# mpc001/auto_avsr

Hardware: AMD Instinct MI355X
Metric: video-frames/sec/node (25fps 88x88, max-frames=1600), E2E training step (fwd+bwd+clip+AdamW) (higher is better)
Workload: dtype f16 activations x f16x2 weights (atrunk3, atrunk4, decoder, encoder, trunk3, trunk4) + split-bf16 (everything else) forward / bf16 backward

## Files before the change

auto_avsr_amd/csrc/loss.hip:

```cpp
#include "prims.h"
#include "avsr_hip.h"
#include "ctc_common.h"

namespace {

AVSR_DEV float log_add(float a, float b) {
    const float m = fmaxf(a, b);
    if (m <= LOG_ZERO) return LOG_ZERO;
    return m + logf(avsr_exp(a - m) + avsr_exp(b - m));
}
AVSR_DEV float log_add3(float a, float b, float c) {
    const float m = fmaxf(a, fmaxf(b, c));
    if (m <= LOG_ZERO) return LOG_ZERO;
    const float sum = avsr_exp(a - m) + avsr_exp(b - m) + avsr_exp(c - m);
#ifdef AVSR_EMU
    return m + logf(sum);
#else
    return m + __logf(sum);
#endif
}

template <class T>
__global__ __launch_bounds__(256) void row_lse_kernel(const T* __restrict__ x, long ld, float* __restrict__ lse,
                                                      long rows, int V) {
// ... 310 lines not shown
    const uint64_t seed = seed0 + (seed_dev ? *seed_dev : 0ull);
    const float inv_keep = p > 0.f ? 1.f / (1.f - p) : 1.f;
    const int dv = D >> 3;
    for (long i = (long)blockIdx.x * 256 + threadIdx.x; i < rows * dv; i += (long)gridDim.x * 256) {
        const long r = i / dv;
        const int c = (int)(i % dv) * 8;
        float e[8], q[8], o[8];
        load8(table + ids[r] * D + c, e);
        load8(pe + (r % L) * D + c, q);
#pragma unroll
        for (int k = 0; k < 8; k++)
            o[k] = (e[k] * scale + q[k]) * dropout_scale(seed, (uint64_t)(r * D + c + k), p, inv_keep);
        store8(out + r * D + c, o);
    }
}
__global__ __launch_bounds__(256) void embed_bwd_kernel(const int64_t* __restrict__ ids, const float* __restrict__ dout,
                                                        float* __restrict__ dtable, long rows, int D, float scale,
                                                        float p, uint64_t seed0, const uint64_t* seed_dev) {
    const uint64_t seed = seed0 + (seed_dev ? *seed_dev : 0ull);
    const float inv_keep = p > 0.f ? 1.f / (1.f - p) : 1.f;
    for (long i = (long)blockIdx.x * 256 + threadIdx.x; i < rows * D; i += (long)gridDim.x * 256) {
        const long r = i / D;
        const int c = (int)(i % D);
        const int64_t id = ids[r];
        bool first = true;
        for (long q = 0; q < r; q++)
            if (ids[q] == id) {
                first = false;
                break;
            }
        if (!first) continue;
        float g = 0.f;
        for (long q = r; q < rows; q++)
// ... 95 lines not shown

extern "C" int avsr_embed_fwd(const int64_t* ids, const float* table, const float* pe, float* out, int64_t rows, int L,
                              int D, float scale, float drop_p, uint64_t seed, const uint64_t* seed_dev, hipStream_t stream) {
    AVSR_REQUIRE(D % 8 == 0, "embed: D must be a multiple of 8");
    if (rows <= 0) return 0;
    long nb = (rows * (D >> 3) + 255) / 256;
    AVSR_LAUNCH(embed_fwd_kernel, dim3((unsigned)(nb > 4096 ? 4096 : nb)), dim3(256), 0, stream, ids, table, pe, out, (long)rows, L, D, scale,
                drop_p, seed, seed_dev);
    AVSR_CHECK_LAUNCH("embed_fwd");
    return 0;
}

extern "C" int avsr_embed_bwd(const int64_t* ids, const float* dout, float* dtable, int64_t rows, int D, float scale,
                              float drop_p, uint64_t seed, const uint64_t* seed_dev, hipStream_t stream) {
    if (rows <= 0) return 0;
    long nb = (rows * D + 255) / 256;
    AVSR_LAUNCH(embed_bwd_kernel, dim3((unsigned)(nb > 4096 ? 4096 : nb)), dim3(256), 0, stream, ids, dout, dtable, (long)rows, D, scale, drop_p,
                seed, seed_dev);
    AVSR_CHECK_LAUNCH("embed_bwd");
    return 0;
}

extern "C" int avsr_log_softmax(const float* x, int64_t ld, float* lse_ws, float* out, int64_t rows, int V,
                                hipStream_t stream) {
    if (rows <= 0) return 0;
    int rc = avsr_row_lse(x, 0, ld, lse_ws, rows, V, stream);
    if (rc) return rc;
    AVSR_LAUNCH(sub_row_scalar_kernel, dim3((unsigned)rows), dim3(256), 0, stream, x, (long)ld, lse_ws, out, (long)rows, V);
    AVSR_CHECK_LAUNCH("log_softmax");
    return 0;
}
```

auto_avsr_amd/csrc/norm.hip:

```cpp
#include "prims.h"
#include "avsr_hip.h"

namespace {

constexpr int LN_THREADS = 256;
constexpr int LN_WAVES = LN_THREADS / 64;
constexpr int LN_MAXV = 4;

template <class TY>
__global__ __launch_bounds__(LN_THREADS) void layernorm_fwd_kernel(
    const float* __restrict__ x, const float* __restrict__ gamma, const float* __restrict__ beta,
    TY* __restrict__ y, float* __restrict__ mean_out, float* __restrict__ rstd_out, int rows,
    int cols, float eps, bf16_t* __restrict__ y2 = nullptr) {
    const int lane = threadIdx.x & 63;
    const int wave = threadIdx.x >> 6;
    const int row = blockIdx.x * LN_WAVES + wave;
    if (row >= rows) return;
    const float* xr = x + (size_t)row * cols;
    const int nvec = cols >> 3;
    float v[LN_MAXV][8];
    float s = 0.f;
#pragma unroll
    for (int i = 0; i < LN_MAXV; i++) {
        const int c = lane + 64 * i;
        if (c < nvec) {
            load8(xr + c * 8, v[i]);
#pragma unroll
            for (int e = 0; e < 8; e++) s += v[i][e];
        }
    }
    const float mean = wave_sum(s) / (float)cols;
    float q = 0.f;
#pragma unroll
    for (int i = 0; i < LN_MAXV; i++) {
        const int c = lane + 64 * i;
        if (c < nvec) {
#pragma unroll
            for (int e = 0; e < 8; e++) {
                const float d = v[i][e] - mean;
                q += d * d;
            }
        }
    }
    const float var = wave_sum(q) / (float)cols;
    const float rstd = 1.0f / sqrtf(var + eps);
    if (lane == 0) {
        mean_out[row] = mean;
        rstd_out[row] = rstd;
    }
    TY* yr = y + (size_t)row * cols;
#pragma unroll
    for (int i = 0; i < LN_MAXV; i++) {
        const int c = lane + 64 * i;
        if (c < nvec) {
            float g[8], b[8], o[8];
            load8(gamma + c * 8, g);
            load8(beta + c * 8, b);
#pragma unroll
            for (int e = 0; e < 8; e++) o[e] = (v[i][e] - mean) * rstd * g[e] + b[e];
            store8(yr + c * 8, o);
            if (y2) store8(y2 + (size_t)row * cols + c * 8, o);
        }
    }
}

template <class TDY>
AVSR_DEV void layernorm_bwd_dx_block(
    const TDY* __restrict__ dy, const float* __restrict__ x, const float* __restrict__ gamma,
    const float* __restrict__ mean_in, const float* __restrict__ rstd_in, const float* __restrict__ dres,
    float* __restrict__ dx, bf16_t* __restrict__ gout, float* __restrict__ gsum, float alpha0, float drop_p, uint64_t seed,
    int rows, int cols, int blk, int rpw, float* red) {
    const int lane = threadIdx.x & 63, wave = threadIdx.x >> 6;
    const int nvec = cols >> 3;
    const float inv_keep = drop_p > 0.f ? 1.f / (1.f - drop_p) : 1.f;
    float pc[LN_MAXV][8];
#pragma unroll
    for (int i = 0; i < LN_MAXV; i++)
#pragma unroll
// ... 171 lines not shown
    if (rows == 0) return 0;
    dim3 grid((rows + LN_WAVES - 1) / LN_WAVES), block(LN_THREADS);
    AVSR_LAUNCH((layernorm_fwd_kernel<float>), grid, block, 0, stream, x, gamma, beta, y, mean, rstd, rows, cols, eps, (bf16_t*)y2);
    AVSR_CHECK_LAUNCH("layernorm_fwd2");
    return 0;
}

extern "C" int avsr_layernorm_fwd_h16(const float* x, const float* gamma, const float* beta, void* y, void* y2, float* mean,
                                      float* rstd, int rows, int cols, float eps, hipStream_t stream) {
    AVSR_REQUIRE(cols % 8 == 0 && cols <= 64 * 8 * LN_MAXV, "layernorm: cols must be %8 and <= 2048");
    if (rows == 0) return 0;
    dim3 grid((rows + LN_WAVES - 1) / LN_WAVES), block(LN_THREADS);
    AVSR_LAUNCH((layernorm_fwd_kernel<f16_t>), grid, block, 0, stream, x, gamma, beta, (f16_t*)y, mean, rstd, rows, cols, eps,
                (bf16_t*)y2);
    AVSR_CHECK_LAUNCH("layernorm_fwd_h16");
    return 0;
}

extern "C" int avsr_layernorm_bwd(const void* dy, int dy_dtype, const float* x, const float* gamma,
                                  const float* mean, const float* rstd, const float* dres, float* dx,
                                  float* dgamma, float* dbeta, void* gout, float* gsum, float alpha, float drop_p,
                                  uint64_t seed, const uint64_t* seed_dev, int rows, int cols, hipStream_t stream) {
    AVSR_REQUIRE(cols % 8 == 0 && cols <= 64 * 8 * LN_MAXV, "layernorm: cols must be %8 and <= 2048");
    AVSR_REQUIRE(gsum == nullptr || gout != nullptr, "layernorm_bwd: gsum needs gout");
    if (rows == 0) return 0;
    float* gsum_det = nullptr;
    if (avsr_det() && gsum) {
        gsum_det = gsum;
        gsum = nullptr;
    }
// ... 20 lines not shown
```

auto_avsr_amd/csrc/optim.hip:

```cpp
#include <math.h>
#include "prims.h"
#include "avsr_hip.h"

namespace {

constexpr int OPT_CHUNK = 4096;

struct OptEntry {
    float* p;
    const float* g;
    float* m;
    float* v;
    long numel;
    int blk0, pad;
};

AVSR_DEV const OptEntry& find_entry(const OptEntry* table, int n, int blk) {
    int lo = 0, hi = n - 1;
    while (lo < hi) {
        const int mid = (lo + hi + 1) >> 1;
        if (table[mid].blk0 <= blk) lo = mid; else hi = mid - 1;
    }
    return table[lo];
}

struct AdamScalars {
    float coef, decay, step_size, inv_sqrt_bc2;
};
AVSR_DEV AdamScalars adam_scalars(const float* state, float beta1, float beta2, float weight_decay) {
    const float step = state[0], lr = state[1];
    const float bc1 = 1.f - powf(beta1, step), bc2 = 1.f - powf(beta2, step);
    return AdamScalars{state[3], 1.f - lr * weight_decay, lr / bc1, 1.f / sqrtf(bc2)};
}
AVSR_DEV void adam_update(float& p, float g, float& m, float& v, const AdamScalars& s, float beta1, float beta2, float eps) {
    const float gk = g * s.coef;
    p *= s.decay;
    m = beta1 * m + (1.f - beta1) * gk;
    v = beta2 * v + (1.f - beta2) * gk * gk;
    const float denom = sqrtf(v) * s.inv_sqrt_bc2 + eps;
// ... 64 lines not shown
        }
    }
}

__global__ __launch_bounds__(64) void grad_window_advance_kernel(float* __restrict__ window, float batch, int close) {
    if (blockIdx.x != 0 || threadIdx.x != 0) return;
    if (close) {
        window[0] = 0.f;
        window[1] = 0.f;
    } else {
        window[0] += 1.f;
        window[1] += batch;
    }
}

__global__ __launch_bounds__(256) void multi_sumsq_kernel(const OptEntry* __restrict__ table, int n, float* __restrict__ partial) {
    __shared__ float red[4];
    const OptEntry e = find_entry(table, n, blockIdx.x);
    const long base = (long)(blockIdx.x - e.blk0) * OPT_CHUNK;
    float s = 0.f;
#pragma unroll
    for (int j = 0; j < 4; j++) {
        const long i = base + (threadIdx.x + 256 * j) * 4;
        if (i + 3 < e.numel && (((uintptr_t)(e.g + i)) & 15) == 0) {
            const f32x4 g = *reinterpret_cast<const f32x4*>(e.g + i);
            s += g[0] * g[0] + g[1] * g[1] + g[2] * g[2] + g[3] * g[3];
        } else {
            for (int k = 0; k < 4; k++)
                if (i + k < e.numel) s += e.g[i + k] * e.g[i + k];
        }
    }
    s = wave_sum(s);
    if ((threadIdx.x & 63) == 0) red[threadIdx.x >> 6] = s;
    __syncthreads();
    if (threadIdx.x == 0) partial[blockIdx.x] = (red[0] + red[1]) + (red[2] + red[3]);
}

__global__ __launch_bounds__(1024) void clip_coef_kernel(const float* __restrict__ partial, int nparts, float max_norm,
                                                        float base_lr, float warmup_steps, float total_steps,
                                                        float* __restrict__ state) {
    __shared__ double red[16];
    double acc[8];
#pragma unroll
    for (int u = 0; u < 8; u++) acc[u] = 0.0;
    for (int i0 = threadIdx.x; i0 < nparts; i0 += 1024 * 8) {
        float v[8];
#pragma unroll
        for (int u = 0; u < 8; u++) v[u] = (i0 + 1024 * u < nparts) ? partial[i0 + 1024 * u] : 0.f;
#pragma unroll
        for (int u = 0; u < 8; u++) acc[u] += (double)v[u];
    }
    double s = ((acc[0] + acc[1]) + (acc[2] + acc[3])) + ((acc[4] + acc[5]) + (acc[6] + acc[7]));
    for (int m = 32; m >= 1; m >>= 1) s += __shfl_xor(s, m);
    if ((threadIdx.x & 63) == 0) red[threadIdx.x >> 6] = s;
    __syncthreads();
    if (threadIdx.x == 0) {
        double tot = 0.0;
        for (int w = 0; w < 16; w++) tot += red[w];
        const float norm = (float)sqrt(tot);
        const float step = state[0] + 1.f;
        float f;
        if (total_steps <= 0.f) f = 1.f;
        else if (step < warmup_steps) f = step / warmup_steps;
// ... 127 lines not shown
        }
#pragma unroll
        for (int k = 0; k < 8; k++) tile[(cc + k) * 72 + r] = f2bf(p[k]);
    }
    __syncthreads();
    if (e.dstT) {
        for (int id = threadIdx.x; id < 64 * 8; id += 256) {
            const int c = id >> 3, rr = (id & 7) * 8;
            const int gc = c0 + c, gr = r0 + rr;
            if (gc < e.C && gr < (e.limT ? e.limT : e.ldT))
                *reinterpret_cast<bf16x8*>(e.dstT + (long)gc * e.ldT + gr) = *reinterpret_cast<const bf16x8*>(tile + c * 72 + rr);
        }
    }
}

}

extern "C" int avsr_adamw_step(const void* table, int n, int total_blocks, float* partial, float* state, float base_lr,
                               float beta1, float beta2, float eps, float weight_decay, float max_grad_norm,
                               int64_t warmup_steps, int64_t total_steps, hipStream_t stream) {
    if (n <= 0 || total_blocks <= 0) return 0;
    AVSR_REQUIRE(table && partial && state, "adamw_step: null argument");
    const OptEntry* t = reinterpret_cast<const OptEntry*>(table);
    AVSR_LAUNCH(multi_sumsq_kernel, dim3(total_blocks), dim3(256), 0, stream, t, n, partial);
    AVSR_LAUNCH(clip_coef_kernel, dim3(1), dim3(1024), 0, stream, (const float*)partial, total_blocks, max_grad_norm, base_lr,
                (float)warmup_steps, (float)total_steps, state);
    AVSR_LAUNCH(multi_adamw_kernel, dim3(total_blocks), dim3(256), 0, stream, t, n, (const float*)state, beta1, beta2, eps,
                weight_decay);
    AVSR_CHECK_LAUNCH("adamw_step");
    return 0;
}

__global__ __launch_bounds__(1024) void sum_partials_kernel(const float* __restrict__ partial, int nparts, float* __restrict__ out) {
    __shared__ double red[16];
    double s = 0.0;
    for (int i = threadIdx.x; i < nparts; i += 1024) s += (double)partial[i];
    for (int m = 32; m >= 1; m >>= 1) s += __shfl_xor(s, m);
    if ((threadIdx.x & 63) == 0) red[threadIdx.x >> 6] = s;
    __syncthreads();
    if (threadIdx.x == 0) {
        double tot = 0.0;
        for (int w = 0; w < 16; w++) tot += red[w];
        out[0] = (float)tot;
    }
}
extern "C" int avsr_multi_sumsq(const void* table, int n, int total_blocks, float* partial, float* sumsq, hipStream_t stream) {
    AVSR_REQUIRE(table && partial && sumsq && n > 0 && total_blocks > 0, "multi_sumsq: bad arguments");
    AVSR_LAUNCH(multi_sumsq_kernel, dim3(total_blocks), dim3(256), 0, stream, reinterpret_cast<const OptEntry*>(table), n, partial);
    AVSR_LAUNCH(sum_partials_kernel, dim3(1), dim3(1024), 0, stream, (const float*)partial, total_blocks, sumsq);
    AVSR_CHECK_LAUNCH("multi_sumsq");
    return 0;
}
extern "C" int avsr_adamw_apply(const void* table, int n, int total_blocks, const float* sumsq, float* state, float base_lr,
                                float beta1, float beta2, float eps, float weight_decay, float max_grad_norm, int64_t warmup_steps,
                                int64_t total_steps, hipStream_t stream) {
    AVSR_REQUIRE(table && sumsq && state && n > 0 && total_blocks > 0, "adamw_apply: bad arguments");
    AVSR_LAUNCH(clip_coef_kernel, dim3(1), dim3(1024), 0, stream, sumsq, 1, max_grad_norm, base_lr, (float)warmup_steps,
                (float)total_steps, state);
    AVSR_LAUNCH(multi_adamw_kernel, dim3(total_blocks), dim3(256), 0, stream, reinterpret_cast<const OptEntry*>(table), n,
                (const float*)state, beta1, beta2, eps, weight_decay);
    AVSR_CHECK_LAUNCH("adamw_apply");
    return 0;
}

extern "C" int avsr_adamw_cast_step(const void* table, int n, int total_blocks, const void* lin_table, int lin_n,
                                    int lin_blocks, const void* tile_table, int tile_n, int tile_blocks, float* partial,
                                    float* state, float base_lr, float beta1, float beta2, float eps, float weight_decay,
                                    float max_grad_norm, int64_t warmup_steps, int64_t total_steps, hipStream_t stream) {
    if (n <= 0 || total_blocks <= 0) return 0;
    AVSR_REQUIRE(table && partial && state, "adamw_cast_step: null argument");
    AVSR_REQUIRE((lin_n <= 0 || lin_table) && (tile_n <= 0 || tile_table), "adamw_cast_step: null table");
    const OptEntry* t = reinterpret_cast<const OptEntry*>(table);
    AVSR_LAUNCH(multi_sumsq_kernel, dim3(total_blocks), dim3(256), 0, stream, t, n, partial);
    AVSR_LAUNCH(clip_coef_kernel, dim3(1), dim3(1024), 0, stream, (const float*)partial, total_blocks, max_grad_norm, base_lr,
                (float)warmup_steps, (float)total_steps, state);
    if (tile_n > 0 && tile_blocks > 0)
        AVSR_LAUNCH(multi_adamw_cast_kernel, dim3(tile_blocks), dim3(256), 0, stream,
                    reinterpret_cast<const OptTileEntry*>(tile_table), tile_n, (const float*)state, beta1, beta2, eps,
                    weight_decay);
    if (lin_n > 0 && lin_blocks > 0)
        AVSR_LAUNCH(multi_adamw_kernel, dim3(lin_blocks), dim3(256), 0, stream, reinterpret_cast<const OptEntry*>(lin_table),
                    lin_n, (const float*)state, beta1, beta2, eps, weight_decay);
    AVSR_CHECK_LAUNCH("adamw_cast_step");
    return 0;
}

extern "C" int avsr_multi_copy_scale(const void* table, int n, int total_blocks, float scale, hipStream_t stream) {
    if (n <= 0 || total_blocks <= 0) return 0;
    AVSR_LAUNCH(multi_copy_scale_kernel, dim3(total_blocks), dim3(256), 0, stream, reinterpret_cast<const OptEntry*>(table), n, scale);
    AVSR_CHECK_LAUNCH("multi_copy_scale");
// ... 14 lines not shown
```

auto_avsr_amd/functional.py:

```python
import contextlib
import os
import math
import struct
import weakref

import torch

from . import ops
from .ops import NN, NT, TN

_state = {"precise": False, "hpf": False, "mixed": False, "f16": False, "wp2": False, "seed": 0x5EED, "counter": 0, "seed_dev": None,
          "bn_sync": None}

MIXED_POLICY = {"encoder": "f16x2", "decoder": "f16x2", "trunk3": "f16x2", "trunk4": "f16x2", "atrunk3": "f16x2", "atrunk4": "f16x2"}
if os.environ.get("AVSR_MIXED_POLICY"):
    MIXED_POLICY = dict(kv.split("=") for kv in os.environ["AVSR_MIXED_POLICY"].split(",") if kv)


def set_precise(flag: bool):
    _state["precise"] = bool(flag)
    _state["hpf"] = _state["mixed"] = _state["f16"] = False
    ops.TWIN = None


# ... 899 lines not shown
    if t2 is None:
        ld = t.stride(-2)
        lead = t.shape[:-1]
        exp = ld
        for size, stride in zip(reversed(lead), reversed(t.stride()[:-1])):
            if size != 1 and stride != exp:
                return None
            exp *= size
        t2 = t.as_strided((rows, n), (ld, 1))
    ld = t2.stride(0)
    if ld % 8 or t2.data_ptr() % 16:
        return None
    return t2, ld


class LayerNormFn(torch.autograd.Function):

    @staticmethod
    def forward(ctx, x, gamma, beta, eps, out_dtype):
        x = x.contiguous()
        ctx.chain = _chain_take(x)
        y, mean, rstd = ops.layernorm_fwd(x, gamma, beta, out_dtype, eps)
        ctx.save_for_backward(x, gamma, mean, rstd)
        return y

    @staticmethod
    @_bwd_mode
    def backward(ctx, dy):
        x, gamma, mean, rstd = ctx.saved_tensors
        D = x.shape[-1]
        dg = _zeros(D, x.device)
        db = _zeros(D, x.device)
        dx = _ln_bwd(dy.contiguous(), x, gamma, mean, rstd, dg, db, None, ctx.chain)
        return dx, dg, db, None, None


def layer_norm(x, gamma, beta, eps=1e-12, out_dtype=torch.float32):
    _state["tag_ok"] = torch.is_grad_enabled()
    return LayerNormFn.apply(_to_f32(x), gamma, beta, eps, out_dtype)


class LinearFn(torch.autograd.Function):

    @staticmethod
    def forward(ctx, x, w, b, out_dtype, pad_out):
        x2 = x.contiguous()
        rows, K = _rows(x2), x2.shape[-1]
        N = w.shape[0]
        ldc = padded_cols(N) if pad_out else N
        alloc = torch.zeros if ldc != N else torch.empty
        y = alloc(x.shape[:-1] + (ldc,), dtype=out_dtype, device=x.device)
        _gemm_nt(x2, w, rows, N, K, y, ldc=ldc, bias=b)
        ctx.save_for_backward(_A(x2), w)
        ctx.meta = (b is not None, x.shape)
# ... 35 lines not shown

def linear(x, w, b=None, out_dtype=None, pad_out=False):
    _state["tag_ok"] = torch.is_grad_enabled()
    return LinearFn.apply(x, w, b, out_dtype or act_dtype(), pad_out)


class FfnSublayerFn(torch.autograd.Function):

    @staticmethod
    def forward(ctx, x, ln_w, ln_b, w1, b1, w2, b2, scale, p, eps):
        x = x.contiguous()
        ctx.chain = _chain_take(x)
        rows, D = _rows(x), x.shape[-1]
        Fh = w1.shape[0]
        T = act_dtype()
        h, mean, rstd = ops.layernorm_fwd(x, ln_w, ln_b, T, eps, twin=True)
        p1, s1, sd1 = _drop_args(p, x)
        u = torch.empty(rows, Fh, dtype=T, device=x.device)
        _gemm_nt(h, w1, rows, Fh, D, u, bias=b1, act=1, drop_p=p1, seed=s1, seed_dev=sd1, twin=True)
        p2, s2, sd2 = _drop_args(p, x)
        y = torch.empty_like(x)
        _gemm_nt(u, w2, rows, D, Fh, y, bias=b2, drop_p=p2, seed=s2, seed_dev=sd2, alpha=scale, resid=x, ldr=D)
        ctx.save_for_backward(x, ln_w, mean, rstd, _A(h), _A(u), w1, w2)
        ctx.meta = (scale, p1, p2, s2, sd2)
        _chain_tag(y, rows, D, scale, (p2, s2, sd2))
        return y

    @staticmethod
    @_bwd_mode
    def backward(ctx, dy):
        x, ln_w, mean, rstd, h, u, w1, w2 = ctx.saved_tensors
# ... 98 lines not shown
        dx = torch.empty(x2.shape, dtype=torch.float32, device=g.device)
        with ops.paired():
            dw1 = _wgrad(du, x2, rows, Fh, Din)
            _gemm_nn(du, w1, rows, Din, Fh, dx)
        return dx, dw1, db1, dw2, db2


def mlp(x, w1, b1, w2, b2):
    _state["tag_ok"] = torch.is_grad_enabled()
    return MlpFn.apply(x, w1, b1, w2, b2)


from .functional_convmod import (
    _const_cache, _const1, _bn_train_stats, _bn_bwd_sums, ConvSublayerFn, conv_sublayer)
from .functional_attention import (
    prepare_pos_proj, _placeholders, _placeholder_grad, PosProjFn, _proj, AttentionCoreFn, attention_core,
    MhaSublayerFn, mha_sublayer, MemoryKVFn, memory_kv)
from .functional_heads import (
    ScaleDropoutFn, scale_dropout, EmbedFn, embed, CtcLossFn, ctc_loss, ctc_align, ctc_beam_search, ctc_score, CeSmoothFn,
    ce_smooth, AddRowsFn, add, log_softmax)
from .functional_frontend import (
    _bn_fwd_params, _bn_bwd, bn_tuple, BasicBlockFn, basic_block, StemFn, stem, AvgPoolFn, avg_pool, trunk_1d)
```

auto_avsr_amd/functional_attention.py:

```python
import math

import torch

from . import functional as AF
from . import ops
from .functional import (
    _A, _A_shared, _A_view, _bgrad, _bias3, _bwd_mode, _chain_tag, _chain_take, _drop_args, _gemm_nn, _gemm_nt,
    _ln_bwd, _mask_arg, _pos_proj, _prologue, _state, _to_act, _to_act_shared, _to_f32, _w_bf16_cat, _w_h16_cat, _h16_nt,
    _wgrad, _zeros, act_dtype)


def prepare_pos_proj(pos_emb, weights):
    _pos_proj.clear()
    if _state["precise"] or len(weights) < 2 or pos_emb is None:
        return
    D = pos_emb.shape[-1]
    if D % 64 or any(w.dtype != torch.float32 or not w.is_contiguous() or tuple(w.shape) != (D, D) for w in weights):
        return
    pe = _to_act_shared(pos_emb).reshape(-1, D)
    if pe.dtype not in (torch.bfloat16, torch.float16):
        return
    n, P = len(weights), pe.shape[0]
    if torch.is_grad_enabled() and all(w.requires_grad for w in weights):
        holder = {}
# ... 13 lines not shown
def _shared_pos_proj(pos_emb, wpos):
    ent = _pos_proj.get(pos_emb, wpos)
    return ent[1] if ent is not None else (None,) * 4


_placeholders = {}


def _placeholder_grad(shape, dtype, device):
    z = _placeholders.get((dtype, device))
    if z is None:
        z = _placeholders[(dtype, device)] = torch.zeros((), dtype=dtype, device=device)
    return z.expand(shape)


class PosProjFn(torch.autograd.Function):

    @staticmethod
    def forward(ctx, pos_emb, holder, *weights):
        D = pos_emb.shape[-1]
        pe = _to_act_shared(pos_emb).reshape(-1, D)
        n, P = len(weights), pe.shape[0]
        out = torch.empty(P, n * D, dtype=pe.dtype, device=pe.device)
        if pe.dtype == torch.float16:
            _h16_nt(pe, D, _w_h16_cat(tuple(weights)), P, n * D, D, out, n * D, planes=1, twin=True)
        else:
            ops.gemm_bf16_nt(pe, D, _w_bf16_cat(tuple(weights), False), D, P, n * D, D, out, n * D)
        ctx.save_for_backward(_A_shared(pe))
        ctx.holder, ctx.meta = holder, (P, D, n)
        return out

    @staticmethod
    @_bwd_mode
    def backward(ctx, dout):
        (pe,) = ctx.saved_tensors
        P, D, n = ctx.meta
        holder = ctx.holder
        assert holder.get("filled", 0) == n and holder.get("dpos") is not None, \
            "PosProjFn: every encoder layer must have accumulated its position gradient"
        dW = _wgrad(holder["dpos"], pe, P, n * D, D)
        holder["dpos"] = None
        holder["filled"] = 0
        return (None, None) + tuple(dW[i * D:(i + 1) * D] for i in range(n))



def _proj(h, w, b, rows, D, twin=True):
    out = torch.empty(rows, w.shape[0], dtype=act_dtype(), device=h.device)
    _gemm_nt(h, w, rows, w.shape[0], D, out, bias=b, twin=twin)
    return out


class AttentionCoreFn(torch.autograd.Function):

    @staticmethod
# ... 376 lines not shown
```

auto_avsr_amd/nets.py:

```python
import math

import torch
from torch import nn

from . import functional as AF
from .scorer_interface import BatchScorerInterface


class LayerNorm(nn.LayerNorm):

    def __init__(self, nout, dim=-1):
        super().__init__(nout, eps=1e-12)
        self.dim = dim

    def forward(self, x):
        if self.dim == -1:
            return AF.layer_norm(x, self.weight, self.bias, self.eps)
        return AF.layer_norm(x.transpose(1, -1), self.weight, self.bias, self.eps).transpose(1, -1)


class PositionwiseFeedForward(nn.Module):

    def __init__(self, idim, hidden_units, dropout_rate):
        super().__init__()
        self.w_1 = nn.Linear(idim, hidden_units)
        self.w_2 = nn.Linear(hidden_units, idim)
        self.dropout = nn.Dropout(dropout_rate)

    def forward(self, x):
        p = self.dropout.p if self.training else 0.0
        return AF.ffn(x, self.w_1.weight, self.w_1.bias, self.w_2.weight, self.w_2.bias, p)

# ... 204 lines not shown
        self.conv_module = conv_module
        self.macaron_style = macaron_style
        self.norm_ff = LayerNorm(size)
        self.norm_mha = LayerNorm(size)
        if macaron_style:
            self.feed_forward_macaron = copy.deepcopy(feed_forward)
            self.ff_scale = 0.5
            self.norm_ff_macaron = LayerNorm(size)
        if conv_module is not None:
            self.norm_conv = LayerNorm(size)
            self.norm_final = LayerNorm(size)
        self.dropout = nn.Dropout(dropout_rate)
        self.size = size
        self.normalize_before = normalize_before
        self.concat_after = concat_after

    def _ffn(self, x, norm, ff):
        p = self.dropout.p if self.training else 0.0
        return AF.ffn_sublayer(x, norm.weight, norm.bias, ff.w_1.weight, ff.w_1.bias, ff.w_2.weight, ff.w_2.bias,
                               self.ff_scale, p, norm.eps)

    def forward(self, x_input, mask, cache=None):
        if cache is not None:
            raise NotImplementedError("incremental encoder cache (dead code in the reference, SURVEY F10)")
        x, pos_emb = x_input if isinstance(x_input, tuple) else (x_input, None)
        p = self.dropout.p if self.training else 0.0
        if self.macaron_style:
            x = self._ffn(x, self.norm_ff_macaron, self.feed_forward_macaron)
        a = self.self_attn
        relpos = pos_emb is not None
        x = AF.mha_sublayer(x, None, pos_emb, mask, self.norm_mha.weight, self.norm_mha.bias, *a._params(),
                            a.linear_pos.weight if relpos else None, a.pos_bias_u if relpos else None,
                            a.pos_bias_v if relpos else None, a.h, a._p_attn(), p, self.norm_mha.eps)
        if self.conv_module is not None:
            x = AF.conv_sublayer(x, self.norm_conv.weight, self.norm_conv.bias, *self.conv_module._params(), p,
                                 self.norm_conv.eps)
        x = self._ffn(x, self.norm_ff, self.feed_forward)
        if self.conv_module is not None:
            x = self.norm_final(x)
        return ((x, pos_emb), mask) if relpos else (x, mask)


def _rename(state_dict, old, new):
    for k in [k for k in state_dict if k.startswith(old)]:
        state_dict[new + k[len(old):]] = state_dict.pop(k)


def _encoder_legacy_keys(state_dict, prefix, *_):
    _rename(state_dict, prefix + "input_layer.", prefix + "embed.")
    _rename(state_dict, prefix + "norm.", prefix + "after_norm.")


class ConformerEncoder(nn.Module):

# ... 5 lines not shown
        self._register_load_state_dict_pre_hook(_encoder_legacy_keys)
        self.embed = nn.Sequential(RelPositionalEncoding(attention_dim, positional_dropout_rate))
        self.normalize_before = normalize_before
        self.encoders = repeat(
            num_blocks,
            lambda n: EncoderLayer(
                attention_dim,
                RelPositionMultiHeadedAttention(attention_heads, attention_dim, attention_dropout_rate, zero_triu),
                PositionwiseFeedForward(attention_dim, linear_units, dropout_rate),
                ConvolutionModule(attention_dim, cnn_module_kernel) if use_cnn_module else None,
                dropout_rate, normalize_before, concat_after, macaron_style),
            layer_drop_rate=0.0,
        )
        if normalize_before:
            self.after_norm = LayerNorm(attention_dim)

    def forward(self, xs, masks):
        with AF.component("encoder"):
            xs = self.embed(xs)
            if isinstance(xs, tuple):
                AF.prepare_pos_proj(xs[1], [layer.self_attn.linear_pos.weight for layer in self.encoders
                                            if hasattr(layer.self_attn, "linear_pos")])
            xs, masks = self.encoders(xs, masks)
            if isinstance(xs, tuple):
                xs = xs[0]
            if self.normalize_before:
                xs = self.after_norm(xs)
        return xs, masks

    def forward_one_step(self, xs, masks, cache=None):
# ... 296 lines not shown
```

auto_avsr_amd/ops.py:

```python
import contextlib
import math
import os

import torch

from . import _lib

F32, BF16, F16 = 0, 1, 2
_DT = {torch.float32: F32, torch.bfloat16: BF16, torch.float16: F16}
NT, NN, TN = 0, 1, 2


def dt(t, split8_ok=False):
    if isinstance(t, Split8):
        if not split8_ok:
            raise TypeError("a split8-layout activation reached an entry point that cannot read it")
        return 3
    return _DT[t.dtype]


def _ptr(t):
    return None if t is None else t.data_ptr()


# ... 91 lines not shown
    y = torch.empty(x.shape, dtype=out_dtype, device=x.device)
    mean = torch.empty(rows, dtype=torch.float32, device=x.device)
    rstd = torch.empty(rows, dtype=torch.float32, device=x.device)
    y2 = _twin(y) if twin else None
    if out_dtype == torch.float16:
        call("avsr_layernorm_fwd_h16", _ptr(x), _ptr(gamma), _ptr(beta), _ptr(y), _ptr(y2), _ptr(mean), _ptr(rstd), rows, cols, eps,
             _stream(x), nbytes=_nb(x, y, y2))
        return y, mean, rstd
    if y2 is not None:
        call("avsr_layernorm_fwd2", _ptr(x), _ptr(gamma), _ptr(beta), _ptr(y), _ptr(y2), _ptr(mean), _ptr(rstd), rows, cols, eps,
             _stream(x), nbytes=_nb(x, y, y2))
        return y, mean, rstd
    call("avsr_layernorm_fwd", _ptr(x), _ptr(gamma), _ptr(beta), _ptr(y), dt(y), _ptr(mean), _ptr(rstd),
         rows, cols, eps, _stream(x), nbytes=_nb(x, y))
    return y, mean, rstd


def layernorm_bwd(dy, x, gamma, mean, rstd, dgamma, dbeta, dres=None, gout=None, gsum=None, alpha=1.0, drop_p=0.0,
                  seed=0, seed_dev=None):
    rows, cols = x.numel() // x.shape[-1], x.shape[-1]
    dx = torch.empty_like(x)
    call("avsr_layernorm_bwd", _ptr(dy), dt(dy), _ptr(x), _ptr(gamma), _ptr(mean), _ptr(rstd), _ptr(dres),
         _ptr(dx), _ptr(dgamma), _ptr(dbeta), _ptr(gout), _ptr(gsum), alpha, drop_p, seed, _ptr(seed_dev), rows, cols,
         _stream(x), nbytes=_nb(dy, x, dres, dx, gout))
    return dx


def gemm(layout, A, lda, B, ldb, M, N, K, C, ldc, *, precise=False, bias=None, act=0, gate=None, ldg=0,
         gate_scale=1.0, drop_p=0.0, seed=0, seed_dev=None, alpha=1.0, alpha_dev=None, resid=None, ldr=0,
         accumulate=False, split_k=1, force_tile=0):
# ... 873 lines not shown
```

include/avsr_hip.h:

```cpp
#ifndef AVSR_HIP_H
#define AVSR_HIP_H
#include <stdint.h>

#if defined(__HIP__) || defined(AVSR_EMU)
typedef hipStream_t avsr_stream_t;
#else
typedef void* avsr_stream_t;
#endif

#ifdef __cplusplus
extern "C" {
#endif

int avsr_abi_version(void);
int avsr_is_emulator(void);
const char* avsr_last_error(void);

int avsr_layernorm_fwd(const float* x, const float* gamma, const float* beta, void* y, int y_dtype,
                       float* mean, float* rstd, int rows, int cols, float eps,
                       avsr_stream_t stream);
int avsr_layernorm_fwd2(const float* x, const float* gamma, const float* beta, float* y, void* y2, float* mean, float* rstd,
                        int rows, int cols, float eps, avsr_stream_t stream);
int avsr_layernorm_bwd(const void* dy, int dy_dtype, const float* x, const float* gamma,
                       const float* mean, const float* rstd, const float* dres, float* dx,
                       float* dgamma, float* dbeta, void* gout, float* gsum, float alpha, float drop_p, uint64_t seed,
                       const uint64_t* seed_dev, int rows, int cols, avsr_stream_t stream);

int avsr_gemm(int layout, const void* A, int a_dtype, int lda, const void* B, int b_dtype, int ldb,
              int M, int N, int K, int precise, const float* bias, int act, const void* gate,
              int gate_dtype, int ldg, float gate_scale, float drop_p, uint64_t seed, const uint64_t* seed_dev,
              float alpha, const float* alpha_dev, const float* resid, int ldr, void* C, int c_dtype, int ldc,
              int accumulate, int split_k, int force_tile, avsr_stream_t stream);

int avsr_attention_fwd(const void* qu, const void* qv, const void* k, const void* v, const void* pos,
                       int dtype, int precise, const uint8_t* mask, int64_t mask_sb, int64_t mask_sq,
                       void* out, float* lse, int B, int H, int Tq, int Tk, int dk, int ldq, int ldk,
                       int ldv, int ldp, int ldo, int64_t sbq, int64_t sbk, int64_t sbv, int64_t sbo,
// ... 342 lines not shown
```

Before: 70520.

## Fuse back-to-back layernorms, rework embed backward and grad-norm reduction

Adds a paired layernorm kernel that computes the encoder layer's final norm and the next layer's macaron FFN norm (or the after_norm) from a single read of the row, handing the second result over through a cache. The embedding backward now has each block build a shared-memory bitmask of rows with matching ids instead of every thread rescanning all earlier ids. The gradient sum-of-squares uses fewer walker blocks that accumulate in double precision. The positional-projection weight gradient casts dpos to bf16 first. These cut launches and redundant memory traffic, at the cost of hand-off state in Python and extra code paths.

```diff
diff --git a/auto_avsr_amd/csrc/loss.hip b/auto_avsr_amd/csrc/loss.hip
--- a/auto_avsr_amd/csrc/loss.hip
+++ b/auto_avsr_amd/csrc/loss.hip
@@ -348,9 +348,61 @@
         store8(out + r * D + c, o);
     }
 }
+constexpr long EMBED_BWD_MAX_ROWS = 32768;
 __global__ __launch_bounds__(256) void embed_bwd_kernel(const int64_t* __restrict__ ids, const float* __restrict__ dout,
                                                         float* __restrict__ dtable, long rows, int D, float scale,
                                                         float p, uint64_t seed0, const uint64_t* seed_dev) {
+    AVSR_DYN_SMEM(smem);
+    const uint64_t seed = seed0 + (seed_dev ? *seed_dev : 0ull);
+    const float inv_keep = p > 0.f ? 1.f / (1.f - p) : 1.f;
+    const int nw = (int)((rows + 63) >> 6);
+    uint64_t* words = reinterpret_cast<uint64_t*>(smem);
+    uint8_t* flag = reinterpret_cast<uint8_t*>(words + nw);
+    for (long r = blockIdx.x; r < rows; r += gridDim.x) {
+        const int64_t id = ids[r];
+        for (int q = threadIdx.x; q < nw * 64; q += 256) flag[q] = (uint8_t)(q < rows && ids[q] == id);
+        __syncthreads();
+        for (int w = threadIdx.x; w < nw; w += 256) {
+            uint64_t m = 0;
+#pragma unroll 8
+            for (int k = 0; k < 64; k++) m |= (uint64_t)flag[w * 64 + k] << k;
+            words[w] = m;
+        }
+        __syncthreads();
+        const int wr = (int)(r >> 6);
+        const uint64_t below = (1ull << (r & 63)) - 1ull;
+        bool first = (words[wr] & below) == 0;
+        for (int w = 0; w < wr && first; w++) first = words[w] == 0;
+        if (first)
+            for (int c = threadIdx.x; c < D; c += 256) {
+                float g = 0.f;
+                for (int w = wr; w < nw; w++) {
+                    uint64_t m = w == wr ? words[w] & ~below : words[w];
+                    while (m) {
+                        long q[4];
+                        float d[4];
+                        int nq = 0;
+#pragma unroll
+                        for (int k = 0; k < 4; k++)
+                            if (m) {
+                                q[nq++] = (long)w * 64 + __builtin_ctzll(m);
+                                m &= m - 1;
+                            }
+#pragma unroll
+                        for (int k = 0; k < 4; k++) d[k] = k < nq ? dout[q[k] * D + c] : 0.f;
+#pragma unroll
+                        for (int k = 0; k < 4; k++)
+                            if (k < nq) g += d[k] * scale * dropout_scale(seed, (uint64_t)(q[k] * D + c), p, inv_keep);
+                    }
+                }
+                dtable[id * D + c] += g;
+            }
+        __syncthreads();
+    }
+}
+__global__ __launch_bounds__(256) void embed_bwd_scan_kernel(const int64_t* __restrict__ ids, const float* __restrict__ dout,
+                                                             float* __restrict__ dtable, long rows, int D, float scale,
+                                                             float p, uint64_t seed0, const uint64_t* seed_dev) {
     const uint64_t seed = seed0 + (seed_dev ? *seed_dev : 0ull);
     const float inv_keep = p > 0.f ? 1.f / (1.f - p) : 1.f;
     for (long i = (long)blockIdx.x * 256 + threadIdx.x; i < rows * D; i += (long)gridDim.x * 256) {
@@ -476,9 +528,15 @@
 extern "C" int avsr_embed_bwd(const int64_t* ids, const float* dout, float* dtable, int64_t rows, int D, float scale,
                               float drop_p, uint64_t seed, const uint64_t* seed_dev, hipStream_t stream) {
     if (rows <= 0) return 0;
-    long nb = (rows * D + 255) / 256;
-    AVSR_LAUNCH(embed_bwd_kernel, dim3((unsigned)(nb > 4096 ? 4096 : nb)), dim3(256), 0, stream, ids, dout, dtable, (long)rows, D, scale, drop_p,
-                seed, seed_dev);
+    if (rows <= EMBED_BWD_MAX_ROWS) {
+        const size_t lds = (size_t)((rows + 63) / 64) * 72;
+        AVSR_LAUNCH(embed_bwd_kernel, dim3((unsigned)(rows > 4096 ? 4096 : rows)), dim3(256), lds, stream, ids, dout, dtable, (long)rows, D,
+                    scale, drop_p, seed, seed_dev);
+    } else {
+        long nb = (rows * D + 255) / 256;
+        AVSR_LAUNCH(embed_bwd_scan_kernel, dim3((unsigned)(nb > 4096 ? 4096 : nb)), dim3(256), 0, stream, ids, dout, dtable, (long)rows, D,
+                    scale, drop_p, seed, seed_dev);
+    }
     AVSR_CHECK_LAUNCH("embed_bwd");
     return 0;
 }
diff --git a/auto_avsr_amd/csrc/norm.hip b/auto_avsr_amd/csrc/norm.hip
--- a/auto_avsr_amd/csrc/norm.hip
+++ b/auto_avsr_amd/csrc/norm.hip
@@ -6,6 +6,57 @@
 constexpr int LN_THREADS = 256;
 constexpr int LN_WAVES = LN_THREADS / 64;
 constexpr int LN_MAXV = 4;
+
+template <class TY, bool KEEP>
+AVSR_DEV void layernorm_row(float (&v)[LN_MAXV][8], int lane, int nvec, int cols, const float* __restrict__ gamma,
+                            const float* __restrict__ beta, float eps, TY* __restrict__ yr, bf16_t* __restrict__ y2r,
+                            float* __restrict__ mean_out, float* __restrict__ rstd_out) {
+    float s = 0.f;
+#pragma unroll
+    for (int i = 0; i < LN_MAXV; i++) {
+        const int c = lane + 64 * i;
+        if (c < nvec) {
+#pragma unroll
+            for (int e = 0; e < 8; e++) s += v[i][e];
+        }
+    }
+    const float mean = wave_sum(s) / (float)cols;
+    float q = 0.f;
+#pragma unroll
+    for (int i = 0; i < LN_MAXV; i++) {
+        const int c = lane + 64 * i;
+        if (c < nvec) {
+#pragma unroll
+            for (int e = 0; e < 8; e++) {
+                const float d = v[i][e] - mean;
+                q += d * d;
+            }
+        }
+    }
+    const float var = wave_sum(q) / (float)cols;
+    const float rstd = 1.0f / sqrtf(var + eps);
+    if (lane == 0) {
+        *mean_out = mean;
+        *rstd_out = rstd;
+    }
+#pragma unroll
+    for (int i = 0; i < LN_MAXV; i++) {
+        const int c = lane + 64 * i;
+        if (c < nvec) {
+            float g[8], b[8], o[8];
+            load8(gamma + c * 8, g);
+            load8(beta + c * 8, b);
+#pragma unroll
+            for (int e = 0; e < 8; e++) o[e] = (v[i][e] - mean) * rstd * g[e] + b[e];
+            store8(yr + c * 8, o);
+            if (y2r) store8(y2r + c * 8, o);
+            if (KEEP) {
+#pragma unroll
+                for (int e = 0; e < 8; e++) v[i][e] = o[e];
+            }
+        }
+    }
+}
 
 template <class TY>
 __global__ __launch_bounds__(LN_THREADS) void layernorm_fwd_kernel(
@@ -19,49 +70,36 @@
     const float* xr = x + (size_t)row * cols;
     const int nvec = cols >> 3;
     float v[LN_MAXV][8];
-    float s = 0.f;
-#pragma unroll
-    for (int i = 0; i < LN_MAXV; i++) {
-        const int c = lane + 64 * i;
-        if (c < nvec) {
-            load8(xr + c * 8, v[i]);
-#pragma unroll
-            for (int e = 0; e < 8; e++) s += v[i][e];
-        }
-    }
-    const float mean = wave_sum(s) / (float)cols;
-    float q = 0.f;
-#pragma unroll
-    for (int i = 0; i < LN_MAXV; i++) {
-        const int c = lane + 64 * i;
-        if (c < nvec) {
-#pragma unroll
-            for (int e = 0; e < 8; e++) {
-                const float d = v[i][e] - mean;
-                q += d * d;
-            }
-        }
-    }
-    const float var = wave_sum(q) / (float)cols;
-    const float rstd = 1.0f / sqrtf(var + eps);
-    if (lane == 0) {
-        mean_out[row] = mean;
-        rstd_out[row] = rstd;
-    }
-    TY* yr = y + (size_t)row * cols;
-#pragma unroll
-    for (int i = 0; i < LN_MAXV; i++) {
-        const int c = lane + 64 * i;
-        if (c < nvec) {
-            float g[8], b[8], o[8];
-            load8(gamma + c * 8, g);
-            load8(beta + c * 8, b);
-#pragma unroll
-            for (int e = 0; e < 8; e++) o[e] = (v[i][e] - mean) * rstd * g[e] + b[e];
-            store8(yr + c * 8, o);
-            if (y2) store8(y2 + (size_t)row * cols + c * 8, o);
-        }
-    }
+#pragma unroll
+    for (int i = 0; i < LN_MAXV; i++) {
+        const int c = lane + 64 * i;
+        if (c < nvec) load8(xr + c * 8, v[i]);
+    }
+    layernorm_row<TY, false>(v, lane, nvec, cols, gamma, beta, eps, y + (size_t)row * cols,
+                             y2 ? y2 + (size_t)row * cols : nullptr, mean_out + row, rstd_out + row);
+}
+
+template <class TH>
+__global__ __launch_bounds__(LN_THREADS) void layernorm_fwd_pair_kernel(
+    const float* __restrict__ x, const float* __restrict__ gamma1, const float* __restrict__ beta1, float* __restrict__ y,
+    float* __restrict__ mean1, float* __restrict__ rstd1, float eps1, const float* __restrict__ gamma2,
+    const float* __restrict__ beta2, TH* __restrict__ h, bf16_t* __restrict__ h2, float* __restrict__ mean2,
+    float* __restrict__ rstd2, float eps2, int rows, int cols) {
+    const int lane = threadIdx.x & 63;
+    const int wave = threadIdx.x >> 6;
+    const int row = blockIdx.x * LN_WAVES + wave;
+    if (row >= rows) return;
+    const float* xr = x + (size_t)row * cols;
+    const int nvec = cols >> 3;
+    float v[LN_MAXV][8];
+#pragma unroll
+    for (int i = 0; i < LN_MAXV; i++) {
+        const int c = lane + 64 * i;
+        if (c < nvec) load8(xr + c * 8, v[i]);
+    }
+    layernorm_row<float, true>(v, lane, nvec, cols, gamma1, beta1, eps1, y + (size_t)row * cols, nullptr, mean1 + row, rstd1 + row);
+    layernorm_row<TH, false>(v, lane, nvec, cols, gamma2, beta2, eps2, h + (size_t)row * cols,
+                             h2 ? h2 + (size_t)row * cols : nullptr, mean2 + row, rstd2 + row);
 }
 
 template <class TDY>
@@ -263,6 +301,26 @@
     AVSR_LAUNCH((layernorm_fwd_kernel<f16_t>), grid, block, 0, stream, x, gamma, beta, (f16_t*)y, mean, rstd, rows, cols, eps,
                 (bf16_t*)y2);
     AVSR_CHECK_LAUNCH("layernorm_fwd_h16");
+    return 0;
+}
+
+extern "C" int avsr_layernorm_fwd_pair(const float* x, const float* gamma1, const float* beta1, float* y, float* mean1, float* rstd1,
+                                       float eps1, const float* gamma2, const float* beta2, void* h, int h_dtype, void* h2,
+                                       float* mean2, float* rstd2, float eps2, int rows, int cols, hipStream_t stream) {
+    AVSR_REQUIRE(cols % 8 == 0 && cols <= 64 * 8 * LN_MAXV, "layernorm: cols must be %8 and <= 2048");
+    AVSR_REQUIRE(h_dtype >= 0 && h_dtype <= 2, "layernorm_fwd_pair: h_dtype is 0 (f32), 1 (bf16) or 2 (f16)");
+    if (rows == 0) return 0;
+    dim3 grid((rows + LN_WAVES - 1) / LN_WAVES), block(LN_THREADS);
+    if (h_dtype == 0)
+        AVSR_LAUNCH((layernorm_fwd_pair_kernel<float>), grid, block, 0, stream, x, gamma1, beta1, y, mean1, rstd1, eps1, gamma2, beta2,
+                    (float*)h, (bf16_t*)h2, mean2, rstd2, eps2, rows, cols);
+    else if (h_dtype == 1)
+        AVSR_LAUNCH((layernorm_fwd_pair_kernel<bf16_t>), grid, block, 0, stream, x, gamma1, beta1, y, mean1, rstd1, eps1, gamma2, beta2,
+                    (bf16_t*)h, (bf16_t*)h2, mean2, rstd2, eps2, rows, cols);
+    else
+        AVSR_LAUNCH((layernorm_fwd_pair_kernel<f16_t>), grid, block, 0, stream, x, gamma1, beta1, y, mean1, rstd1, eps1, gamma2, beta2,
+                    (f16_t*)h, (bf16_t*)h2, mean2, rstd2, eps2, rows, cols);
+    AVSR_CHECK_LAUNCH("layernorm_fwd_pair");
     return 0;
 }
 
diff --git a/auto_avsr_amd/csrc/optim.hip b/auto_avsr_amd/csrc/optim.hip
--- a/auto_avsr_amd/csrc/optim.hip
+++ b/auto_avsr_amd/csrc/optim.hip
@@ -15,14 +15,15 @@
     int blk0, pad;
 };
 
-AVSR_DEV const OptEntry& find_entry(const OptEntry* table, int n, int blk) {
+AVSR_DEV int find_index(const OptEntry* table, int n, int blk) {
     int lo = 0, hi = n - 1;
     while (lo < hi) {
         const int mid = (lo + hi + 1) >> 1;
         if (table[mid].blk0 <= blk) lo = mid; else hi = mid - 1;
     }
-    return table[lo];
-}
+    return lo;
+}
+AVSR_DEV const OptEntry& find_entry(const OptEntry* table, int n, int blk) { return table[find_index(table, n, blk)]; }
 
 struct AdamScalars {
     float coef, decay, step_size, inv_sqrt_bc2;
@@ -117,29 +118,55 @@
     }
 }
 
+AVSR_DEV float chunk_sumsq(const float* __restrict__ g, long numel, long base) {
+    float s = 0.f;
+#pragma unroll
+    for (int j = 0; j < 4; j++) {
+        const long i = base + (threadIdx.x + 256 * j) * 4;
+        if (i + 3 < numel && (((uintptr_t)(g + i)) & 15) == 0) {
+            const f32x4 v = *reinterpret_cast<const f32x4*>(g + i);
+            s += v[0] * v[0] + v[1] * v[1] + v[2] * v[2] + v[3] * v[3];
+        } else {
+            for (int k = 0; k < 4; k++)
+                if (i + k < numel) s += g[i + k] * g[i + k];
+        }
+    }
+    return s;
+}
+
 __global__ __launch_bounds__(256) void multi_sumsq_kernel(const OptEntry* __restrict__ table, int n, float* __restrict__ partial) {
     __shared__ float red[4];
     const OptEntry e = find_entry(table, n, blockIdx.x);
-    const long base = (long)(blockIdx.x - e.blk0) * OPT_CHUNK;
-    float s = 0.f;
-#pragma unroll
-    for (int j = 0; j < 4; j++) {
-        const long i = base + (threadIdx.x + 256 * j) * 4;
-        if (i + 3 < e.numel && (((uintptr_t)(e.g + i)) & 15) == 0) {
-            const f32x4 g = *reinterpret_cast<const f32x4*>(e.g + i);
-            s += g[0] * g[0] + g[1] * g[1] + g[2] * g[2] + g[3] * g[3];
-        } else {
-            for (int k = 0; k < 4; k++)
-                if (i + k < e.numel) s += e.g[i + k] * e.g[i + k];
-        }
-    }
+    float s = chunk_sumsq(e.g, e.numel, (long)(blockIdx.x - e.blk0) * OPT_CHUNK);
     s = wave_sum(s);
     if ((threadIdx.x & 63) == 0) red[threadIdx.x >> 6] = s;
     __syncthreads();
     if (threadIdx.x == 0) partial[blockIdx.x] = (red[0] + red[1]) + (red[2] + red[3]);
 }
 
-__global__ __launch_bounds__(1024) void clip_coef_kernel(const float* __restrict__ partial, int nparts, float max_norm,
+constexpr int SUMSQ_WALKERS = 2048;
+__global__ __launch_bounds__(256) void multi_sumsq_walk_kernel(const OptEntry* __restrict__ table, int n, int total_blocks,
+                                                               double* __restrict__ partial) {
+    __shared__ double red[4];
+    const int per = (total_blocks + (int)gridDim.x - 1) / (int)gridDim.x;
+    const int b0 = (int)blockIdx.x * per;
+    const int b1 = b0 + per < total_blocks ? b0 + per : total_blocks;
+    double s = 0.0;
+    if (b0 < b1) {
+        int idx = find_index(table, n, b0);
+        for (int blk = b0; blk < b1; blk++) {
+            while (idx + 1 < n && table[idx + 1].blk0 <= blk) idx++;
+            s += (double)chunk_sumsq(table[idx].g, table[idx].numel, (long)(blk - table[idx].blk0) * OPT_CHUNK);
+        }
+    }
+    for (int m = 32; m >= 1; m >>= 1) s += __shfl_xor(s, m);
+    if ((threadIdx.x & 63) == 0) red[threadIdx.x >> 6] = s;
+    __syncthreads();
+    if (threadIdx.x == 0) partial[blockIdx.x] = (red[0] + red[1]) + (red[2] + red[3]);
+}
+
+template <typename T>
+__global__ __launch_bounds__(1024) void clip_coef_kernel(const T* __restrict__ partial, int nparts, float max_norm,
                                                         float base_lr, float warmup_steps, float total_steps,
                                                         float* __restrict__ state) {
     __shared__ double red[16];
@@ -147,9 +174,9 @@
 #pragma unroll
     for (int u = 0; u < 8; u++) acc[u] = 0.0;
     for (int i0 = threadIdx.x; i0 < nparts; i0 += 1024 * 8) {
-        float v[8];
-#pragma unroll
-        for (int u = 0; u < 8; u++) v[u] = (i0 + 1024 * u < nparts) ? partial[i0 + 1024 * u] : 0.f;
+        T v[8];
+#pragma unroll
+        for (int u = 0; u < 8; u++) v[u] = (i0 + 1024 * u < nparts) ? partial[i0 + 1024 * u] : (T)0;
 #pragma unroll
         for (int u = 0; u < 8; u++) acc[u] += (double)v[u];
     }
@@ -307,6 +334,26 @@
     }
 }
 
+int launch_sumsq(const OptEntry* t, int n, int total_blocks, float* partial, hipStream_t stream, bool* wide) {
+    *wide = total_blocks >= 2 && (((uintptr_t)partial) & 7) == 0;
+    if (!*wide) {
+        AVSR_LAUNCH(multi_sumsq_kernel, dim3(total_blocks), dim3(256), 0, stream, t, n, partial);
+        return total_blocks;
+    }
+    const int grid = total_blocks / 2 < SUMSQ_WALKERS ? total_blocks / 2 : SUMSQ_WALKERS;
+    AVSR_LAUNCH(multi_sumsq_walk_kernel, dim3(grid), dim3(256), 0, stream, t, n, total_blocks, reinterpret_cast<double*>(partial));
+    return grid;
+}
+void launch_clip_coef(const float* partial, int nparts, bool wide, float max_grad_norm, float base_lr, int64_t warmup_steps,
+                      int64_t total_steps, float* state, hipStream_t stream) {
+    if (wide)
+        AVSR_LAUNCH(clip_coef_kernel<double>, dim3(1), dim3(1024), 0, stream, reinterpret_cast<const double*>(partial), nparts,
+                    max_grad_norm, base_lr, (float)warmup_steps, (float)total_steps, state);
+    else
+        AVSR_LAUNCH(clip_coef_kernel<float>, dim3(1), dim3(1024), 0, stream, partial, nparts, max_grad_norm, base_lr,
+                    (float)warmup_steps, (float)total_steps, state);
+}
+
 }
 
 extern "C" int avsr_adamw_step(const void* table, int n, int total_blocks, float* partial, float* state, float base_lr,
@@ -315,16 +362,17 @@
     if (n <= 0 || total_blocks <= 0) return 0;
     AVSR_REQUIRE(table && partial && state, "adamw_step: null argument");
     const OptEntry* t = reinterpret_cast<const OptEntry*>(table);
-    AVSR_LAUNCH(multi_sumsq_kernel, dim3(total_blocks), dim3(256), 0, stream, t, n, partial);
-    AVSR_LAUNCH(clip_coef_kernel, dim3(1), dim3(1024), 0, stream, (const float*)partial, total_blocks, max_grad_norm, base_lr,
-                (float)warmup_steps, (float)total_steps, state);
+    bool wide;
+    const int nparts = launch_sumsq(t, n, total_blocks, partial, stream, &wide);
+    launch_clip_coef(partial, nparts, wide, max_grad_norm, base_lr, warmup_steps, total_steps, state, stream);
     AVSR_LAUNCH(multi_adamw_kernel, dim3(total_blocks), dim3(256), 0, stream, t, n, (const float*)state, beta1, beta2, eps,
                 weight_decay);
     AVSR_CHECK_LAUNCH("adamw_step");
     return 0;
 }
 
-__global__ __launch_bounds__(1024) void sum_partials_kernel(const float* __restrict__ partial, int nparts, float* __restrict__ out) {
+template <typename T>
+__global__ __launch_bounds__(1024) void sum_partials_kernel(const T* __restrict__ partial, int nparts, float* __restrict__ out) {
     __shared__ double red[16];
     double s = 0.0;
     for (int i = threadIdx.x; i < nparts; i += 1024) s += (double)partial[i];
@@ -339,8 +387,10 @@
 }
 extern "C" int avsr_multi_sumsq(const void* table, int n, int total_blocks, float* partial, float* sumsq, hipStream_t stream) {
     AVSR_REQUIRE(table && partial && sumsq && n > 0 && total_blocks > 0, "multi_sumsq: bad arguments");
-    AVSR_LAUNCH(multi_sumsq_kernel, dim3(total_blocks), dim3(256), 0, stream, reinterpret_cast<const OptEntry*>(table), n, partial);
-    AVSR_LAUNCH(sum_partials_kernel, dim3(1), dim3(1024), 0, stream, (const float*)partial, total_blocks, sumsq);
+    bool wide;
+    const int nparts = launch_sumsq(reinterpret_cast<const OptEntry*>(table), n, total_blocks, partial, stream, &wide);
+    if (wide) AVSR_LAUNCH(sum_partials_kernel<double>, dim3(1), dim3(1024), 0, stream, reinterpret_cast<const double*>(partial), nparts, sumsq);
+    else AVSR_LAUNCH(sum_partials_kernel<float>, dim3(1), dim3(1024), 0, stream, (const float*)partial, nparts, sumsq);
     AVSR_CHECK_LAUNCH("multi_sumsq");
     return 0;
 }
@@ -348,8 +398,7 @@
                                 float beta1, float beta2, float eps, float weight_decay, float max_grad_norm, int64_t warmup_steps,
                                 int64_t total_steps, hipStream_t stream) {
     AVSR_REQUIRE(table && sumsq && state && n > 0 && total_blocks > 0, "adamw_apply: bad arguments");
-    AVSR_LAUNCH(clip_coef_kernel, dim3(1), dim3(1024), 0, stream, sumsq, 1, max_grad_norm, base_lr, (float)warmup_steps,
-                (float)total_steps, state);
+    launch_clip_coef(sumsq, 1, false, max_grad_norm, base_lr, warmup_steps, total_steps, state, stream);
     AVSR_LAUNCH(multi_adamw_kernel, dim3(total_blocks), dim3(256), 0, stream, reinterpret_cast<const OptEntry*>(table), n,
                 (const float*)state, beta1, beta2, eps, weight_decay);
     AVSR_CHECK_LAUNCH("adamw_apply");
@@ -364,9 +413,9 @@
     AVSR_REQUIRE(table && partial && state, "adamw_cast_step: null argument");
     AVSR_REQUIRE((lin_n <= 0 || lin_table) && (tile_n <= 0 || tile_table), "adamw_cast_step: null table");
     const OptEntry* t = reinterpret_cast<const OptEntry*>(table);
-    AVSR_LAUNCH(multi_sumsq_kernel, dim3(total_blocks), dim3(256), 0, stream, t, n, partial);
-    AVSR_LAUNCH(clip_coef_kernel, dim3(1), dim3(1024), 0, stream, (const float*)partial, total_blocks, max_grad_norm, base_lr,
-                (float)warmup_steps, (float)total_steps, state);
+    bool wide;
+    const int nparts = launch_sumsq(t, n, total_blocks, partial, stream, &wide);
+    launch_clip_coef(partial, nparts, wide, max_grad_norm, base_lr, warmup_steps, total_steps, state, stream);
     if (tile_n > 0 && tile_blocks > 0)
         AVSR_LAUNCH(multi_adamw_cast_kernel, dim3(tile_blocks), dim3(256), 0, stream,
                     reinterpret_cast<const OptTileEntry*>(tile_table), tile_n, (const float*)state, beta1, beta2, eps,
diff --git a/auto_avsr_amd/functional.py b/auto_avsr_amd/functional.py
--- a/auto_avsr_amd/functional.py
+++ b/auto_avsr_amd/functional.py
@@ -937,13 +937,29 @@
     return t2, ld
 
 
+_LN_PAIR = os.environ.get("AVSR_LN_PAIR", "1") != "0"
+_ln_pair = _HandOff("ln_pair", 8)
+
+
+def _ln_fwd(x, gamma, beta, out_dtype, eps, twin=False):
+    ent = _ln_pair.pop(x, gamma, beta, extra=(float(eps), out_dtype, bool(twin))) if len(_ln_pair) else None
+    if ent is not None and ent[0][0].shape == x.shape:
+        return ent[1]
+    return ops.layernorm_fwd(x, gamma, beta, out_dtype, eps, twin=twin)
+
+
 class LayerNormFn(torch.autograd.Function):
 
     @staticmethod
-    def forward(ctx, x, gamma, beta, eps, out_dtype):
+    def forward(ctx, x, gamma, beta, eps, out_dtype, then):
         x = x.contiguous()
         ctx.chain = _chain_take(x)
-        y, mean, rstd = ops.layernorm_fwd(x, gamma, beta, out_dtype, eps)
+        if then is not None and _LN_PAIR and out_dtype == torch.float32 and then[0].shape == gamma.shape:
+            g2, b2, eps2, dt2, twin2 = then
+            (y, mean, rstd), second = ops.layernorm_fwd_pair(x, gamma, beta, eps, g2, b2, eps2, dt2, twin=twin2)
+            _ln_pair.put(second, y, g2, b2, extra=(float(eps2), dt2, bool(twin2)))
+        else:
+            y, mean, rstd = _ln_fwd(x, gamma, beta, out_dtype, eps)
         ctx.save_for_backward(x, gamma, mean, rstd)
         return y
 
@@ -955,12 +971,15 @@
         dg = _zeros(D, x.device)
         db = _zeros(D, x.device)
         dx = _ln_bwd(dy.contiguous(), x, gamma, mean, rstd, dg, db, None, ctx.chain)
-        return dx, dg, db, None, None
-
-
-def layer_norm(x, gamma, beta, eps=1e-12, out_dtype=torch.float32):
+        return dx, dg, db, None, None, None
+
+
+def layer_norm(x, gamma, beta, eps=1e-12, out_dtype=torch.float32, then=None):
     _state["tag_ok"] = torch.is_grad_enabled()
-    return LayerNormFn.apply(_to_f32(x), gamma, beta, eps, out_dtype)
+    if then is not None:
+        kind, g2, b2, eps2 = then
+        then = (g2, b2, eps2, act_dtype(), True) if kind == "ffn" else (g2, b2, eps2, torch.float32, False)
+    return LayerNormFn.apply(_to_f32(x), gamma, beta, eps, out_dtype, then)
 
 
 class LinearFn(torch.autograd.Function):
@@ -1026,7 +1045,7 @@
         rows, D = _rows(x), x.shape[-1]
         Fh = w1.shape[0]
         T = act_dtype()
-        h, mean, rstd = ops.layernorm_fwd(x, ln_w, ln_b, T, eps, twin=True)
+        h, mean, rstd = _ln_fwd(x, ln_w, ln_b, T, eps, twin=True)
         p1, s1, sd1 = _drop_args(p, x)
         u = torch.empty(rows, Fh, dtype=T, device=x.device)
         _gemm_nt(h, w1, rows, Fh, D, u, bias=b1, act=1, drop_p=p1, seed=s1, seed_dev=sd1, twin=True)
@@ -1155,7 +1174,7 @@
 from .functional_convmod import (
     _const_cache, _const1, _bn_train_stats, _bn_bwd_sums, ConvSublayerFn, conv_sublayer)
 from .functional_attention import (
-    prepare_pos_proj, _placeholders, _placeholder_grad, PosProjFn, _proj, AttentionCoreFn, attention_core,
+    prepare_pos_proj, _placeholders, _placeholder_grad, _pos_wgrad, PosProjFn, _proj, AttentionCoreFn, attention_core,
     MhaSublayerFn, mha_sublayer, MemoryKVFn, memory_kv)
 from .functional_heads import (
     ScaleDropoutFn, scale_dropout, EmbedFn, embed, CtcLossFn, ctc_loss, ctc_align, ctc_beam_search, ctc_score, CeSmoothFn,
diff --git a/auto_avsr_amd/functional_attention.py b/auto_avsr_amd/functional_attention.py
--- a/auto_avsr_amd/functional_attention.py
+++ b/auto_avsr_amd/functional_attention.py
@@ -51,6 +51,12 @@
     return z.expand(shape)
 
 
+def _pos_wgrad(dpos, pe, P, n_out, D):
+    if not _state["precise"] and dpos.dtype == torch.float32 and pe.dtype == torch.bfloat16 and n_out % 8 == 0 and D % 8 == 0:
+        dpos = ops.scale_dropout(dpos, torch.bfloat16)
+    return _wgrad(dpos, pe, P, n_out, D)
+
+
 class PosProjFn(torch.autograd.Function):
 
     @staticmethod
@@ -75,7 +81,7 @@
         holder = ctx.holder
         assert holder.get("filled", 0) == n and holder.get("dpos") is not None, \
             "PosProjFn: every encoder layer must have accumulated its position gradient"
-        dW = _wgrad(holder["dpos"], pe, P, n * D, D)
+        dW = _pos_wgrad(holder["dpos"], pe, P, n * D, D)
         holder["dpos"] = None
         holder["filled"] = 0
         return (None, None) + tuple(dW[i * D:(i + 1) * D] for i in range(n))
diff --git a/auto_avsr_amd/nets.py b/auto_avsr_amd/nets.py
--- a/auto_avsr_amd/nets.py
+++ b/auto_avsr_amd/nets.py
@@ -13,9 +13,11 @@
         super().__init__(nout, eps=1e-12)
         self.dim = dim
 
-    def forward(self, x):
+    def forward(self, x, then=None):
         if self.dim == -1:
-            return AF.layer_norm(x, self.weight, self.bias, self.eps)
+            if then is not None:
+                then = (then[0], then[1].weight, then[1].bias, then[1].eps)
+            return AF.layer_norm(x, self.weight, self.bias, self.eps, then=then)
         return AF.layer_norm(x.transpose(1, -1), self.weight, self.bias, self.eps).transpose(1, -1)
 
 
@@ -250,6 +252,7 @@
         self.size = size
         self.normalize_before = normalize_before
         self.concat_after = concat_after
+        self.next_norm = None
 
     def _ffn(self, x, norm, ff):
         p = self.dropout.p if self.training else 0.0
@@ -273,7 +276,7 @@
                                  self.norm_conv.eps)
         x = self._ffn(x, self.norm_ff, self.feed_forward)
         if self.conv_module is not None:
-            x = self.norm_final(x)
+            x = self.norm_final(x, then=self.next_norm)
         return ((x, pos_emb), mask) if relpos else (x, mask)
 
 
@@ -309,6 +312,12 @@
         )
         if normalize_before:
             self.after_norm = LayerNorm(attention_dim)
+        layers = list(self.encoders)
+        for cur, nxt in zip(layers, layers[1:]):
+            if macaron_style:
+                cur.next_norm = ("ffn", nxt.norm_ff_macaron)
+        if normalize_before and layers:
+            layers[-1].next_norm = ("norm", self.after_norm)
 
     def forward(self, xs, masks):
         with AF.component("encoder"):
diff --git a/auto_avsr_amd/ops.py b/auto_avsr_amd/ops.py
--- a/auto_avsr_amd/ops.py
+++ b/auto_avsr_amd/ops.py
@@ -129,6 +129,18 @@
     call("avsr_layernorm_fwd", _ptr(x), _ptr(gamma), _ptr(beta), _ptr(y), dt(y), _ptr(mean), _ptr(rstd),
          rows, cols, eps, _stream(x), nbytes=_nb(x, y))
     return y, mean, rstd
+
+
+def layernorm_fwd_pair(x, gamma1, beta1, eps1, gamma2, beta2, eps2, h_dtype, twin=False):
+    rows, cols = x.numel() // x.shape[-1], x.shape[-1]
+    y = torch.empty(x.shape, dtype=torch.float32, device=x.device)
+    h = torch.empty(x.shape, dtype=h_dtype, device=x.device)
+    st = [torch.empty(rows, dtype=torch.float32, device=x.device) for _ in range(4)]
+    h2 = _twin(h) if twin else None
+    call("avsr_layernorm_fwd_pair", _ptr(x), _ptr(gamma1), _ptr(beta1), _ptr(y), _ptr(st[0]), _ptr(st[1]), eps1, _ptr(gamma2),
+         _ptr(beta2), _ptr(h), {torch.float32: 0, torch.bfloat16: 1, torch.float16: 2}[h_dtype], _ptr(h2), _ptr(st[2]), _ptr(st[3]),
+         eps2, rows, cols, _stream(x), nbytes=_nb(x, y, h, h2))
+    return (y, st[0], st[1]), (h, st[2], st[3])
 
 
 def layernorm_bwd(dy, x, gamma, mean, rstd, dgamma, dbeta, dres=None, gout=None, gsum=None, alpha=1.0, drop_p=0.0,
diff --git a/include/avsr_hip.h b/include/avsr_hip.h
--- a/include/avsr_hip.h
+++ b/include/avsr_hip.h
@@ -21,6 +21,9 @@
                        avsr_stream_t stream);
 int avsr_layernorm_fwd2(const float* x, const float* gamma, const float* beta, float* y, void* y2, float* mean, float* rstd,
                         int rows, int cols, float eps, avsr_stream_t stream);
+int avsr_layernorm_fwd_pair(const float* x, const float* gamma1, const float* beta1, float* y, float* mean1, float* rstd1,
+                            float eps1, const float* gamma2, const float* beta2, void* h, int h_dtype, void* h2, float* mean2,
+                            float* rstd2, float eps2, int rows, int cols, avsr_stream_t stream);
 int avsr_layernorm_bwd(const void* dy, int dy_dtype, const float* x, const float* gamma,
                        const float* mean, const float* rstd, const float* dres, float* dx,
                        float* dgamma, float* dbeta, void* gout, float* gsum, float alpha, float drop_p, uint64_t seed,
```

Result: no change. 70430 (-0.1%).
